# ai-dynamo/grove

Measured on AMD Instinct MI355X. Metric: podgangs_per_sec, higher is better.
Workload: dtype bf16; 1 GPU; global_batch=4, parallelism=gang1, gang_size=1, payload=2048x2048x2048x1, inflight=2, concurrent_syncs=4, transport=http, scheduler=amd-gang-scheduler (native xGMI Filter/Score)

## Files before the change

### grove_amd/kubelet/gpunode.py

```python
from __future__ import annotations

import logging
from typing import Any, Dict, Optional, Tuple

from ..api import constants as c
from ..kubecore.store import Obj

log = logging.getLogger("grove.gpunode")

PAYLOAD_ANNOTATION = "grove.io/payload"
PAYLOAD_SHAPE_ANNOTATION = "grove.io/payload-shape"
GPU_IDS_ANNOTATION = "scheduling.amd.com/gpu-ids"

_gpuwork = None


def load_gpuwork():
    global _gpuwork
    if _gpuwork is not None:
        return _gpuwork
    import torch
    try:
        from ..ops import _gpuwork as ext
    except ImportError as e:
        if torch.cuda.is_available():
            raise RuntimeError(
                "grove_amd.ops._gpuwork native extension is missing on a GPU box — "
                "build it with python -m grove_amd.ops.build") from e
        return None
    _gpuwork = ext
    return ext


PAYLOAD_KINDS = ("gemm", "stream", "decode", "decode_batch", "decode_attn")


def parse_payload_shape(kind: str, shape: str) -> Tuple[int, ...]:
    if kind == "gemm":
        dims = tuple(int(x) for x in shape.split("x")) if shape else (1024, 1024, 1024, 1)
        if len(dims) == 3:
            dims = dims + (1,)
        return dims
    if kind == "stream":
        dims = tuple(int(v) for v in shape.split("x")) if shape else (1 << 24,)
        if len(dims) == 1:
            dims = dims + (2,)
        return dims
    if kind == "decode":
        dims = tuple(int(v) for v in shape.split("x")) if shape else (8192, 8192, 4)
        if len(dims) == 2:
            dims = dims + (1,)
        return dims
    if kind == "decode_batch":
        dims = tuple(int(v) for v in shape.split("x")) if shape else (16384, 8192, 16, 4)
        if len(dims) == 3:
            dims = dims + (1,)
        if len(dims) != 4:
            raise ValueError(
                f"decode_batch payload-shape must be NxKxB[xiters], got {shape!r}")
        return dims
    if kind == "decode_attn":
        dims = tuple(int(v) for v in shape.split("x")) if shape else (64, 8, 8192, 32, 4)
        if len(dims) == 4:
            dims = dims + (1,)
        if len(dims) != 5:
            raise ValueError(
                f"decode_attn payload-shape must be HQxHKVxCTXxB[xiters], got {shape!r}")
        return dims
    raise ValueError(f"unknown payload kind {kind!r}")


def parse_payload(pod: Obj) -> Tuple[str, Tuple[int, ...]]:
    ann = pod["metadata"].get("annotations") or {}
    kind = ann.get(PAYLOAD_ANNOTATION, "gemm")
    shape = ann.get(PAYLOAD_SHAPE_ANNOTATION, "")
    if kind in PAYLOAD_KINDS:
        return kind, parse_payload_shape(kind, shape)
    return "none", ()


def assigned_gpu(pod: Obj) -> Optional[int]:
    ids = (pod["metadata"].get("annotations") or {}).get(GPU_IDS_ANNOTATION, "")
    if not ids:
        return None
    return int(ids.split(",")[0])


def run_payload_descriptor(kind: str, dims: Tuple[int, ...], device: int) -> Dict[str, Any]:
    import torch
    if not torch.cuda.is_available():
        if kind == "gemm":
            m, n, k, iters = dims
            a = torch.randn(min(m, 128), min(k, 128))
            b = torch.randn(min(k, 128), min(n, 128))
            for _ in range(iters):
                a @ b
        return {"device": "cpu", "kind": kind}
    ext = load_gpuwork()
    device = device % max(1, torch.cuda.device_count())
    with torch.cuda.device(device):
        if kind == "gemm":
            m, n, k, iters = dims
            tflops = ext.burn_gemm(m, n, k, iters)
            return {"device": device, "kind": kind, "tflops": tflops}
        if kind == "stream":
            n_floats = dims[0]
            iters = dims[1] if len(dims) > 1 else 2
            gbps = ext.stream_triad(n_floats, iters)
            return {"device": device, "kind": kind, "gbps": gbps}
        if kind == "decode":
            n, k, iters = dims
            gbps = ext.burn_decode(n, k, iters)
            return {"device": device, "kind": kind, "weight_stream_gbps": gbps}
        if kind == "decode_batch":
            n, k, batch, iters = dims
            gbps = ext.burn_decode_batch(n, k, batch, iters)
            return {"device": device, "kind": kind, "batch": batch,
                    "weight_stream_gbps": gbps,
                    "tokens_per_s": batch * gbps * 1e9 / (2.0 * n * k)}
        if kind == "decode_attn":
            hq, hkv, ctx, batch, iters = dims
            gbps = ext.burn_decode_attn(hq, hkv, ctx, batch, iters)
            kv_bytes_per_step = 2.0 * batch * hkv * ctx * 128 * 2
            return {"device": device, "kind": kind, "batch": batch, "context": ctx,
                    "kv_stream_gbps": gbps,
                    "tokens_per_s": batch * gbps * 1e9 / kv_bytes_per_step}
    return {"device": device, "kind": kind}


def gpu_pod_payload(pod: Obj) -> None:
    gpu = assigned_gpu(pod)
    kind, dims = parse_payload(pod)
    if kind == "none":
        return
    if gpu is None:
        gpu = 0
    run_payload_descriptor(kind, dims, gpu)
```

### grove_amd/ops/gpuwork.hip

```cpp
#include <torch/extension.h>
#include <ATen/hip/HIPContext.h>
#include <hip/hip_runtime.h>
#include <hip/hip_bf16.h>

#include <vector>

#define WAVE 64
#define BK 64

using bf16 = __hip_bfloat16;
using bf16x8 = __attribute__((ext_vector_type(8))) __bf16;
using f32x16 = __attribute__((ext_vector_type(16))) float;

__device__ __forceinline__ int swz(int row, int cb) {
    return (cb ^ ((row ^ (row >> 3)) & 7)) & 7;
}

__device__ __forceinline__ int lds_off(int row, int cb) {
    return row * BK + (swz(row, cb) << 3);
}

__device__ __forceinline__ void tile_map(int bid, int num_pid_m, int tiles_n,
                                         int& tile_m, int& tile_n) {
    const int GROUP = 8;
    int group_size = min(GROUP, num_pid_m);
    int pids_per_group = group_size * tiles_n;
    int group = bid / pids_per_group;
    int in_group = bid % pids_per_group;
    tile_m = group * GROUP + (in_group % group_size);
    tile_n = in_group / group_size;
}

__device__ __forceinline__ void tile_map_rect(int bid, int tiles_m, int tiles_n,
                                              int m_per_xcd, int n_win,
                                              int& tile_m, int& tile_n) {
    int mwin_tiles = 8 * m_per_xcd;
    int win = bid >> 8;
    int idx = bid & 255;
    int xcd = idx & 7;
    int slot = idx >> 3;
    int nwins = tiles_n / n_win;
    tile_m = (win / nwins) * mwin_tiles + xcd * m_per_xcd + slot % m_per_xcd;
    tile_n = (win % nwins) * n_win + slot / m_per_xcd;
}

template <int THREADS, int AUX = 0>
__device__ __forceinline__ void stage_tile(const bf16* __restrict__ g, long ld,
                                           __bf16* __restrict__ dst, int rows,
                                           int tid, int wave_piece0) {
#pragma unroll
    for (int i = 0; i < 8; ++i) {
        if (i >= (rows * 8) / THREADS)
            break;
        int p = tid + i * THREADS;
        int row = p >> 3;
        int cb_src = swz(row, p & 7);
        int base = wave_piece0 + i * THREADS;
        __builtin_amdgcn_global_load_lds(
            (const __attribute__((address_space(1))) uint32_t*)(
                g + (long)row * ld + (cb_src << 3)),
            (__attribute__((address_space(3))) uint32_t*)(dst + base * 8),
            16, 0, AUX);
    }
}

__global__ __launch_bounds__(512, 1)
void mfma_gemm_bf16_256_kernel(const bf16* __restrict__ A,
                               const bf16* __restrict__ Bt,
                               float* __restrict__ C,
                               int M, int N, int K,
                               int m_per_xcd, int n_win) {
    constexpr int BM = 256, BN = 256;
    __shared__ __bf16 smem[2 * (BM * BK + BN * BK)];
    auto sAp = [&](int b) { return smem + b * (BM * BK + BN * BK); };
    auto sBp = [&](int b) { return smem + b * (BM * BK + BN * BK) + BM * BK; };

    int tile_m, tile_n;
    if (m_per_xcd)
        tile_map_rect(blockIdx.x, M / BM, N / BN, m_per_xcd, n_win,
                      tile_m, tile_n);
    else
        tile_map(blockIdx.x, M / BM, N / BN, tile_m, tile_n);
    const int tid = threadIdx.x;
    const int wave = tid / WAVE;
    const int lane = tid % WAVE;
    const int wr = wave >> 1, wc = wave & 1;
    const long row0 = (long)tile_m * BM;
    const long col0 = (long)tile_n * BN;
    const int wave_piece0 = wave * WAVE;

    auto stage = [&](int buf, long kk) {
        stage_tile<512>(A + row0 * K + kk, K, sAp(buf), BM, tid, wave_piece0);
        stage_tile<512>(Bt + col0 * K + kk, K, sBp(buf), BN, tid, wave_piece0);
    };

    f32x16 acc[2][4] = {};
    bf16x8 afrag[2][2], bfrag[2][4];
    const int a_row = wr * 64 + (lane & 31);
    const int b_row = wc * 128 + (lane & 31);
    const int k_half = lane >> 5;
    auto load_frags = [&](int pb, int buf, int ks) {
        int cb = (ks << 1) | k_half;
#pragma unroll
        for (int mt = 0; mt < 2; ++mt)
            afrag[pb][mt] = *(const bf16x8*)(sAp(buf) + lds_off(a_row + mt * 32, cb));
#pragma unroll
        for (int nt = 0; nt < 4; ++nt)
            bfrag[pb][nt] = *(const bf16x8*)(sBp(buf) + lds_off(b_row + nt * 32, cb));
    };

    stage(0, 0);
    __syncthreads();
    load_frags(0, 0, 0);
    for (long kk = 0; kk < K; kk += BK) {
        int buf = (kk / BK) & 1;
        if (kk + BK < K) stage(buf ^ 1, kk + BK);
#pragma unroll
        for (int ks = 0; ks < BK / 16; ++ks) {
            int pb = ks & 1;
            if (ks + 1 < BK / 16)
                load_frags(pb ^ 1, buf, ks + 1);
#pragma unroll
            for (int mt = 0; mt < 2; ++mt)
#pragma unroll
                for (int nt = 0; nt < 4; ++nt)
                    acc[mt][nt] = __builtin_amdgcn_mfma_f32_32x32x16_bf16(
                        afrag[pb][mt], bfrag[pb][nt], acc[mt][nt], 0, 0, 0);
        }
        __syncthreads();
        if (kk + BK < K) load_frags(0, buf ^ 1, 0);
    }

    const int c_row_lane = 4 * (lane >> 5);
#pragma unroll
    for (int mt = 0; mt < 2; ++mt)
#pragma unroll
        for (int nt = 0; nt < 4; ++nt)
#pragma unroll
            for (int reg = 0; reg < 16; ++reg) {
                int r = wr * 64 + mt * 32 + (reg & 3) + 8 * (reg >> 2) + c_row_lane;
                int cl = wc * 128 + nt * 32 + (lane & 31);
                C[(row0 + r) * (long)N + col0 + cl] = acc[mt][nt][reg];
            }
}

__global__ __launch_bounds__(256, 2)
void mfma_gemm_bf16_128_kernel(const bf16* __restrict__ A,
                               const bf16* __restrict__ Bt,
                               float* __restrict__ C,
                               int M, int N, int K) {
    constexpr int BM = 128, BN = 128;
    __shared__ __bf16 smem[2 * (BM * BK + BN * BK)];
    auto sAp = [&](int b) { return smem + b * (BM * BK + BN * BK); };
    auto sBp = [&](int b) { return smem + b * (BM * BK + BN * BK) + BM * BK; };

    int tile_m, tile_n;
    tile_map(blockIdx.x, M / BM, N / BN, tile_m, tile_n);
    const int tid = threadIdx.x;
    const int wave = tid / WAVE;
    const int lane = tid % WAVE;
    const int wr = wave >> 1, wc = wave & 1;
    const long row0 = (long)tile_m * BM;
    const long col0 = (long)tile_n * BN;
    const int wave_piece0 = wave * WAVE;

    auto stage = [&](int buf, long kk) {
        stage_tile<256>(A + row0 * K + kk, K, sAp(buf), BM, tid, wave_piece0);
        stage_tile<256>(Bt + col0 * K + kk, K, sBp(buf), BN, tid, wave_piece0);
    };

    f32x16 acc[2][2] = {};
    bf16x8 afrag[2][2], bfrag[2][2];
    const int a_row = wr * 64 + (lane & 31);
    const int b_row = wc * 64 + (lane & 31);
    const int k_half = lane >> 5;
    auto load_frags = [&](int pb, int buf, int ks) {
        int cb = (ks << 1) | k_half;
#pragma unroll
        for (int mt = 0; mt < 2; ++mt)
            afrag[pb][mt] = *(const bf16x8*)(sAp(buf) + lds_off(a_row + mt * 32, cb));
#pragma unroll
        for (int nt = 0; nt < 2; ++nt)
            bfrag[pb][nt] = *(const bf16x8*)(sBp(buf) + lds_off(b_row + nt * 32, cb));
    };

    stage(0, 0);
    __syncthreads();
    load_frags(0, 0, 0);
    for (long kk = 0; kk < K; kk += BK) {
        int buf = (kk / BK) & 1;
        if (kk + BK < K) stage(buf ^ 1, kk + BK);
#pragma unroll
        for (int ks = 0; ks < BK / 16; ++ks) {
            int pb = ks & 1;
            if (ks + 1 < BK / 16)
                load_frags(pb ^ 1, buf, ks + 1);
#pragma unroll
            for (int mt = 0; mt < 2; ++mt)
#pragma unroll
                for (int nt = 0; nt < 2; ++nt)
                    acc[mt][nt] = __builtin_amdgcn_mfma_f32_32x32x16_bf16(
                        afrag[pb][mt], bfrag[pb][nt], acc[mt][nt], 0, 0, 0);
        }
        __syncthreads();
        if (kk + BK < K) load_frags(0, buf ^ 1, 0);
    }

    const int c_row_lane = 4 * (lane >> 5);
#pragma unroll
    for (int mt = 0; mt < 2; ++mt)
#pragma unroll
        for (int nt = 0; nt < 2; ++nt)
#pragma unroll
            for (int reg = 0; reg < 16; ++reg) {
                int r = wr * 64 + mt * 32 + (reg & 3) + 8 * (reg >> 2) + c_row_lane;
                int cl = wc * 64 + nt * 32 + (lane & 31);
                C[(row0 + r) * (long)N + col0 + cl] = acc[mt][nt][reg];
            }
}

__global__ __launch_bounds__(256)
void decode_gemv_kernel(const bf16* __restrict__ W,
                        const bf16* __restrict__ x,
                        float* __restrict__ y, int N, int K) {
    const int lane = threadIdx.x % WAVE;
    const int wave = threadIdx.x / WAVE;
    const int row = blockIdx.x * 4 + wave;
    if (row >= N) return;
    const bf16* w = W + (long)row * K;
    float acc = 0.f;
    for (int k0 = lane * 8; k0 < K; k0 += WAVE * 8) {
        bf16x8 wv = *(const bf16x8*)(w + k0);
        bf16x8 xv = *(const bf16x8*)(x + k0);
#pragma unroll
        for (int i = 0; i < 8; ++i)
            acc += (float)wv[i] * (float)xv[i];
    }
    for (int off = 32; off > 0; off >>= 1)
        acc += __shfl_down(acc, off, 64);
    if (lane == 0) y[row] = acc;
}

torch::Tensor decode_gemv(torch::Tensor w, torch::Tensor x) {
    TORCH_CHECK(w.is_cuda() && x.is_cuda() && w.dtype() == torch::kBFloat16
                && x.dtype() == torch::kBFloat16, "bf16 GPU tensors required");
    TORCH_CHECK(w.is_contiguous() && x.is_contiguous(), "contiguous required");
    int64_t N = w.size(0), K = w.size(1);
    TORCH_CHECK(x.numel() == K && K % 512 == 0, "x must be [K], K%512==0");
    auto y = torch::empty({N}, w.options().dtype(torch::kFloat32));
    hipStream_t stream = at::hip::getCurrentHIPStream();
    hipLaunchKernelGGL(decode_gemv_kernel, dim3((N + 3) / 4), dim3(256), 0, stream,
                       (const bf16*)w.data_ptr(), (const bf16*)x.data_ptr(),
                       y.data_ptr<float>(), (int)N, (int)K);
    return y;
}

double burn_decode(int64_t n, int64_t k, int64_t iters) {
    auto opt = torch::TensorOptions().dtype(torch::kBFloat16).device(torch::kCUDA);
    auto w = torch::randn({n, k}, opt.dtype(torch::kFloat32)).to(torch::kBFloat16);
    auto x = torch::randn({k}, opt.dtype(torch::kFloat32)).to(torch::kBFloat16);
    auto y = torch::empty({n}, opt.dtype(torch::kFloat32));
    hipStream_t stream = at::hip::getCurrentHIPStream();
    auto launch = [&] {
        hipLaunchKernelGGL(decode_gemv_kernel, dim3((n + 3) / 4), dim3(256), 0,
                           stream, (const bf16*)w.data_ptr(),
                           (const bf16*)x.data_ptr(), y.data_ptr<float>(),
                           (int)n, (int)k);
    };
    launch();
    C10_HIP_CHECK(hipStreamSynchronize(stream));
    auto t0 = std::chrono::steady_clock::now();
    for (int64_t i = 0; i < iters; ++i) launch();
    C10_HIP_CHECK(hipStreamSynchronize(stream));
    auto t1 = std::chrono::steady_clock::now();
    double secs = std::chrono::duration<double>(t1 - t0).count();
    return 2.0 * n * k * iters / secs / 1e9;
}

using f32x4 = __attribute__((ext_vector_type(4))) float;

#define DG_STEP 128

template <int T, int R>
__global__ __launch_bounds__(256)
void decode_gemm_kernel(const bf16* __restrict__ W,
                        const bf16* __restrict__ X,
                        float* __restrict__ Y,
                        int B, int N, int K) {
    __shared__ f32x4 red[4 * R * T * WAVE];
    const int lane = threadIdx.x % WAVE;
    const int wave = threadIdx.x / WAVE;
    const int r = lane & 15, g = lane >> 4;
    const int kq = K / 4;
    const int steps = kq / DG_STEP;
    const long koff = (long)wave * kq + 8 * g;
    const long n0 = (long)blockIdx.x * (16 * R);
    const bf16* wp = W + (n0 + r) * K + koff;
    const auto xrsrc = __builtin_amdgcn_make_buffer_rsrc(
        const_cast<bf16*>(X), 0, B * K * 2, 0x00020000);
    unsigned xoff[T];
#pragma unroll
    for (int t = 0; t < T; ++t)
        xoff[t] = (unsigned)(((long)(t * 16 + r) * K + koff) * 2);

    auto load_w = [&](bf16x8 (&w)[R][4], int s) {
#pragma unroll
        for (int q = 0; q < R; ++q) {
            const bf16x8* p = (const bf16x8*)(wp + (long)q * 16 * K + (long)s * DG_STEP);
#pragma unroll
            for (int i = 0; i < 4; ++i)
                w[q][i] = p[4 * i];
        }
    };
    auto load_x = [&](bf16x8 (&x)[T][4], int s) {
#pragma unroll
        for (int t = 0; t < T; ++t)
#pragma unroll
            for (int i = 0; i < 4; ++i)
                x[t][i] = __builtin_bit_cast(bf16x8, __builtin_amdgcn_raw_buffer_load_b128(
                    xrsrc, xoff[t] + s * (DG_STEP * 2) + i * 64, 0, 0));
    };

    f32x4 acc[R][T] = {};
    auto mma = [&](const bf16x8 (&w)[R][4], const bf16x8 (&x)[T][4]) {
#pragma unroll
        for (int i = 0; i < 4; ++i)
#pragma unroll
            for (int q = 0; q < R; ++q)
#pragma unroll
                for (int t = 0; t < T; ++t)
                    acc[q][t] = __builtin_amdgcn_mfma_f32_16x16x32_bf16(
                        w[q][i], x[t][i], acc[q][t], 0, 0, 0);
    };

    bf16x8 w0[R][4], w1[R][4], xf[T][4];
    load_w(w0, 0);
    int s = 0;
    for (; s + 2 < steps; s += 2) {
        load_x(xf, s);
        load_w(w1, s + 1);
        mma(w0, xf);
        load_x(xf, s + 1);
        load_w(w0, s + 2);
        mma(w1, xf);
    }
    load_x(xf, s);
    if (s + 1 < steps) {
        load_w(w1, s + 1);
        mma(w0, xf);
        load_x(xf, s + 1);
        mma(w1, xf);
    } else {
        mma(w0, xf);
    }

#pragma unroll
    for (int q = 0; q < R; ++q)
#pragma unroll
        for (int t = 0; t < T; ++t)
            red[((wave * R + q) * T + t) * WAVE + lane] = acc[q][t];
    __syncthreads();
    const int nl = threadIdx.x & 15, bl = threadIdx.x >> 4;
    const float* redf = (const float*)red;
    const int src = (((nl >> 2) * 16 + bl) << 2) + (nl & 3);
#pragma unroll
    for (int q = 0; q < R; ++q)
#pragma unroll
        for (int t = 0; t < T; ++t) {
            int b = t * 16 + bl;
            if (b < B) {
                float sum = redf[(q * T + t) * WAVE * 4 + src];
#pragma unroll
                for (int w = 1; w < 4; ++w)
                    sum += redf[((w * R + q) * T + t) * WAVE * 4 + src];
                Y[(long)b * N + n0 + q * 16 + nl] = sum;
            }
        }
}

static void check_decode_gemm_dims(int64_t B, int64_t N, int64_t K) {
    TORCH_CHECK(B >= 1 && B <= 64 && N >= 16 && N % 16 == 0 && K >= 512 && K % 512 == 0
                && N <= INT32_MAX && K <= (1 << 23),
                "decode_gemm_bf16 requires 1<=B<=64, N%16==0, K%512==0 (got B=", B,
                " N=", N, " K=", K, ")");
}

template <int T>
static void launch_decode_gemm_t(const bf16* w, const bf16* x, float* y, int B, int N,
                                 int K, int rows, hipStream_t stream) {
    dim3 grid(N / (16 * rows)), block(256);
    auto go = [&](auto kernel) {
        hipLaunchKernelGGL(kernel, grid, block, 0, stream, w, x, y, B, N, K);
    };
    if (rows == 4) go(decode_gemm_kernel<T, 4>);
    else if (rows == 2) go(decode_gemm_kernel<T, 2>);
    else go(decode_gemm_kernel<T, 1>);
}

static int decode_gemm_rows(int64_t B, int64_t N) {
    int rows = B <= 8 ? 1 : B <= 16 ? 2 : 4;
    while (rows > 1 && (N % (16 * rows) != 0 || N / (16 * rows) < 256))
        rows /= 2;
    return rows;
}

static void launch_decode_gemm(const bf16* w, const bf16* x, float* y, int64_t B,
                               int64_t N, int64_t K, int64_t rows, hipStream_t stream) {
    if (!rows) rows = decode_gemm_rows(B, N);
    TORCH_CHECK((rows == 1 || rows == 2 || rows == 4) && N % (16 * rows) == 0,
                "rows must be 0 (auto), 1, 2 or 4 and 16*rows must divide N");
    switch ((B + 15) / 16) {
    case 1: launch_decode_gemm_t<1>(w, x, y, B, N, K, rows, stream); break;
    case 2: launch_decode_gemm_t<2>(w, x, y, B, N, K, rows, stream); break;
    case 3: launch_decode_gemm_t<3>(w, x, y, B, N, K, rows, stream); break;
    default: launch_decode_gemm_t<4>(w, x, y, B, N, K, rows, stream); break;
    }
}

torch::Tensor decode_gemm_bf16(torch::Tensor w, torch::Tensor x) {
    TORCH_CHECK(w.is_cuda() && x.is_cuda() && w.dtype() == torch::kBFloat16
                && x.dtype() == torch::kBFloat16, "bf16 GPU tensors required");
    TORCH_CHECK(w.get_device() == x.get_device(), "w and x must be on one device");
    TORCH_CHECK(w.dim() == 2 && x.dim() == 2, "w must be [N,K] and x [B,K]");
    TORCH_CHECK(w.is_contiguous() && x.is_contiguous(), "contiguous required");
    int64_t N = w.size(0), K = w.size(1), B = x.size(0);
    TORCH_CHECK(x.size(1) == K, "shape mismatch: w[N,K] x[B,K]");
    check_decode_gemm_dims(B, N, K);
    auto y = torch::empty({B, N}, w.options().dtype(torch::kFloat32));
    launch_decode_gemm((const bf16*)w.data_ptr(), (const bf16*)x.data_ptr(),
                       y.data_ptr<float>(), B, N, K, 0,
                       at::hip::getCurrentHIPStream());
    return y;
}

double burn_decode_batch(int64_t n, int64_t k, int64_t batch, int64_t iters,
                         int64_t rows) {
    check_decode_gemm_dims(batch, n, k);
    auto opt = torch::TensorOptions().dtype(torch::kBFloat16).device(torch::kCUDA);
    auto w = torch::randn({n, k}, opt.dtype(torch::kFloat32)).to(torch::kBFloat16);
    auto x = torch::randn({batch, k}, opt.dtype(torch::kFloat32)).to(torch::kBFloat16);
    auto y = torch::empty({batch, n}, opt.dtype(torch::kFloat32));
    hipStream_t stream = at::hip::getCurrentHIPStream();
    auto launch = [&] {
        launch_decode_gemm((const bf16*)w.data_ptr(), (const bf16*)x.data_ptr(),
                           y.data_ptr<float>(), batch, n, k, rows, stream);
    };
    launch();
    C10_HIP_CHECK(hipStreamSynchronize(stream));
    auto t0 = std::chrono::steady_clock::now();
    for (int64_t i = 0; i < iters; ++i) launch();
    C10_HIP_CHECK(hipStreamSynchronize(stream));
    auto t1 = std::chrono::steady_clock::now();
    double secs = std::chrono::duration<double>(t1 - t0).count();
    return 2.0 * n * k * iters / secs / 1e9;
}

__global__ void stream_triad_kernel(const float4* __restrict__ a,
                                    const float4* __restrict__ b,
                                    float4* __restrict__ c, long n4, float s) {
    long i = (long)blockIdx.x * blockDim.x + threadIdx.x;
    long stride = (long)gridDim.x * blockDim.x;
    for (; i < n4; i += stride) {
        float4 x = a[i], y = b[i];
        c[i] = make_float4(x.x + s * y.x, x.y + s * y.y, x.z + s * y.z, x.w + s * y.w);
    }
}


static void launch_gemm(const torch::Tensor& a, const torch::Tensor& bt,
                        torch::Tensor& c, int64_t M, int64_t N, int64_t K,
                        int64_t map_mode = -1) {
    hipStream_t stream = at::hip::getCurrentHIPStream();
    if (M % 256 == 0 && N % 256 == 0 && (M / 256) * (N / 256) >= 256) {
        int tiles_m = (int)(M / 256), tiles_n = (int)(N / 256);
        int m_per_xcd = 0, n_win = 0;
        int mpx = std::min<int>(4, std::max(1, tiles_m / 8));
        int nw = 256 / (8 * mpx);
        bool want_rect = (map_mode == 1) ||
                         (map_mode < 0 && (int64_t)tiles_m * tiles_n > 256);
        if (want_rect && map_mode != 0 &&
            tiles_m % (8 * mpx) == 0 && tiles_n % nw == 0) {
            m_per_xcd = mpx; n_win = nw;
        }
        dim3 grid((M / 256) * (N / 256)), block(512);
        hipLaunchKernelGGL(mfma_gemm_bf16_256_kernel, grid, block, 0, stream,
                           (const bf16*)a.data_ptr(), (const bf16*)bt.data_ptr(),
                           c.data_ptr<float>(), (int)M, (int)N, (int)K,
                           m_per_xcd, n_win);
    } else {
        dim3 grid((M / 128) * (N / 128)), block(256);
        hipLaunchKernelGGL(mfma_gemm_bf16_128_kernel, grid, block, 0, stream,
                           (const bf16*)a.data_ptr(), (const bf16*)bt.data_ptr(),
                           c.data_ptr<float>(), (int)M, (int)N, (int)K);
    }
}

static void check_dims(int64_t M, int64_t N, int64_t K) {
    TORCH_CHECK(M % 128 == 0 && N % 128 == 0 && K % 64 == 0,
                "mfma_gemm_bf16 requires M%128==0, N%128==0, K%64==0 (got ",
                M, "x", N, "x", K, ")");
}

torch::Tensor mfma_gemm_bf16(torch::Tensor a, torch::Tensor bt) {
    TORCH_CHECK(a.is_cuda() && bt.is_cuda(), "inputs must be on GPU");
    TORCH_CHECK(a.dtype() == torch::kBFloat16 && bt.dtype() == torch::kBFloat16,
                "inputs must be bf16");
    TORCH_CHECK(a.is_contiguous() && bt.is_contiguous(), "inputs must be contiguous");
    int64_t M = a.size(0), K = a.size(1), N = bt.size(0);
    TORCH_CHECK(bt.size(1) == K, "shape mismatch: A[M,K] Bt[N,K]");
    check_dims(M, N, K);
    auto c = torch::empty({M, N}, a.options().dtype(torch::kFloat32));
    launch_gemm(a, bt, c, M, N, K);
    return c;
}

double burn_gemm(int64_t m, int64_t n, int64_t k, int64_t iters,
                 int64_t map_mode) {
    check_dims(m, n, k);
    auto opt = torch::TensorOptions().dtype(torch::kBFloat16).device(torch::kCUDA);
    auto a = torch::randn({m, k}, opt.dtype(torch::kFloat32)).to(torch::kBFloat16);
    auto bt = torch::randn({n, k}, opt.dtype(torch::kFloat32)).to(torch::kBFloat16);
    auto c = torch::empty({m, n}, opt.dtype(torch::kFloat32));
    hipStream_t stream = at::hip::getCurrentHIPStream();
    launch_gemm(a, bt, c, m, n, k, map_mode);
    C10_HIP_CHECK(hipStreamSynchronize(stream));
    auto t0 = std::chrono::steady_clock::now();
    for (int64_t i = 0; i < iters; ++i) launch_gemm(a, bt, c, m, n, k, map_mode);
    C10_HIP_CHECK(hipStreamSynchronize(stream));
    auto t1 = std::chrono::steady_clock::now();
    double secs = std::chrono::duration<double>(t1 - t0).count();
    return 2.0 * m * n * k * iters / secs / 1e12;
}

double stream_triad(int64_t n_floats, int64_t iters) {
    TORCH_CHECK(n_floats % 4 == 0, "n_floats must be a multiple of 4");
    auto opt = torch::TensorOptions().dtype(torch::kFloat32).device(torch::kCUDA);
    auto a = torch::randn({n_floats}, opt);
    auto b = torch::randn({n_floats}, opt);
    auto c = torch::empty({n_floats}, opt);
    long n4 = n_floats / 4;
    hipStream_t stream = at::hip::getCurrentHIPStream();
    int blocks = std::min<long>(8192, (n4 + 255) / 256);
    auto launch = [&] {
        hipLaunchKernelGGL(stream_triad_kernel, dim3(blocks), dim3(256), 0, stream,
                           (const float4*)a.data_ptr(), (const float4*)b.data_ptr(),
                           (float4*)c.data_ptr(), n4, 1.5f);
    };
    launch();
    C10_HIP_CHECK(hipStreamSynchronize(stream));
    auto t0 = std::chrono::steady_clock::now();
    for (int64_t i = 0; i < iters; ++i) launch();
    C10_HIP_CHECK(hipStreamSynchronize(stream));
    auto t1 = std::chrono::steady_clock::now();
    double secs = std::chrono::duration<double>(t1 - t0).count();
    return 12.0 * n_floats * iters / secs / 1e9;
}

torch::Tensor decode_attn_bf16(torch::Tensor q, torch::Tensor k_cache,
                               torch::Tensor v_cache, torch::Tensor seq_lens,
                               double scale, int64_t splits);
int64_t decode_attn_splits(int64_t batch, int64_t hkv, int64_t lmax);
double burn_decode_attn(int64_t hq, int64_t hkv, int64_t ctx, int64_t batch,
                        int64_t iters, int64_t splits);

PYBIND11_MODULE(TORCH_EXTENSION_NAME, m) {
    m.doc() = "grove_amd MI355X pod-payload kernels (MFMA bf16 GEMM, HBM stream, "
              "decode GEMV, batched decode skinny GEMM, split-KV decode attention)";
    m.def("mfma_gemm_bf16", &mfma_gemm_bf16, "C[M,N]=A[M,K]@Bt[N,K]^T (bf16 in, fp32 out)");
    m.def("burn_gemm", &burn_gemm, "run iters GEMM steps; returns TFLOP/s",
          pybind11::arg("m"), pybind11::arg("n"), pybind11::arg("k"),
          pybind11::arg("iters"), pybind11::arg("map_mode") = -1);
    m.def("burn_gemm_v",
          [](int64_t m_, int64_t n_, int64_t k_, int64_t it, int64_t) {
              return burn_gemm(m_, n_, k_, it, -1);
          }, "compat alias for burn_gemm (bk arg ignored)");
    m.def("stream_triad", &stream_triad, "HBM triad; returns GB/s");
    m.def("decode_gemv", &decode_gemv, "y[N]=W[N,K]@x[K] (bf16 in, fp32 out)");
    m.def("burn_decode", &burn_decode,
          "iters decode GEMV steps; returns weight-stream GB/s");
    m.def("decode_gemm_bf16", &decode_gemm_bf16,
          "y[B,N]=x[B,K]@W[N,K]^T for 1<=B<=64, N%16==0, K%512==0 "
          "(args w, x; bf16 in, fp32 out)");
    m.def("burn_decode_batch", &burn_decode_batch,
          "iters batched decode steps; returns weight-stream GB/s",
          pybind11::arg("n"), pybind11::arg("k"), pybind11::arg("batch"),
          pybind11::arg("iters"), pybind11::arg("rows") = 0);
    m.def("decode_attn_bf16", &decode_attn_bf16,
          "out[B,Hq,128]=softmax(scale*q.k^T).v over k/v_cache[B,Hkv,Lmax,128] up to "
          "seq_lens[B] (int32, on device); bf16 in, fp32 out; scale=0 -> 1/sqrt(128); "
          "splits=0 -> automatic",
          pybind11::arg("q"), pybind11::arg("k_cache"), pybind11::arg("v_cache"),
          pybind11::arg("seq_lens"), pybind11::arg("scale") = 0.0,
          pybind11::arg("splits") = 0);
    m.def("decode_attn_splits", &decode_attn_splits,
          "KV splits decode_attn_bf16 picks for a shape",
          pybind11::arg("batch"), pybind11::arg("hkv"), pybind11::arg("lmax"));
    m.def("burn_decode_attn", &burn_decode_attn,
          "iters decode-attention steps; returns KV-stream GB/s",
          pybind11::arg("hq"), pybind11::arg("hkv"), pybind11::arg("ctx"),
          pybind11::arg("batch"), pybind11::arg("iters"), pybind11::arg("splits") = 0);
}
```

Measured before the change: 358.4 gangs/s.

## Run pod payloads in native code with fused fill, no warmup, GIL released

Adds native payload entry points for gemm, decode and decode_batch. Each one fills both operands with a single counter-hash bf16 kernel into one shared buffer, runs the iterations without a warmup launch, and synchronises once. These calls release the GIL and pick the device with a C++ guard instead of the Python torch.cuda.device context. The aim is to drop the torch.randn plus cast kernels, the warmup GEMM and the extra syncs, and to let concurrent pod syncs overlap. In exchange the input distribution changes from normal to uniform, and timing now includes the fill.

Measured after the change: 332.2 gangs/s. 7.3% lower.

```diff
diff --git a/grove_amd/kubelet/gpunode.py b/grove_amd/kubelet/gpunode.py
--- a/grove_amd/kubelet/gpunode.py
+++ b/grove_amd/kubelet/gpunode.py
@@ -98,26 +98,26 @@
         return {"device": "cpu", "kind": kind}
     ext = load_gpuwork()
     device = device % max(1, torch.cuda.device_count())
+    if kind == "gemm":
+        m, n, k, iters = dims
+        tflops = ext.gemm_payload(m, n, k, iters, device)
+        return {"device": device, "kind": kind, "tflops": tflops}
+    if kind == "decode":
+        n, k, iters = dims
+        gbps = ext.decode_payload(n, k, iters, device)
+        return {"device": device, "kind": kind, "weight_stream_gbps": gbps}
+    if kind == "decode_batch":
+        n, k, batch, iters = dims
+        gbps = ext.decode_batch_payload(n, k, batch, iters, device)
+        return {"device": device, "kind": kind, "batch": batch,
+                "weight_stream_gbps": gbps,
+                "tokens_per_s": batch * gbps * 1e9 / (2.0 * n * k)}
     with torch.cuda.device(device):
-        if kind == "gemm":
-            m, n, k, iters = dims
-            tflops = ext.burn_gemm(m, n, k, iters)
-            return {"device": device, "kind": kind, "tflops": tflops}
         if kind == "stream":
             n_floats = dims[0]
             iters = dims[1] if len(dims) > 1 else 2
             gbps = ext.stream_triad(n_floats, iters)
             return {"device": device, "kind": kind, "gbps": gbps}
-        if kind == "decode":
-            n, k, iters = dims
-            gbps = ext.burn_decode(n, k, iters)
-            return {"device": device, "kind": kind, "weight_stream_gbps": gbps}
-        if kind == "decode_batch":
-            n, k, batch, iters = dims
-            gbps = ext.burn_decode_batch(n, k, batch, iters)
-            return {"device": device, "kind": kind, "batch": batch,
-                    "weight_stream_gbps": gbps,
-                    "tokens_per_s": batch * gbps * 1e9 / (2.0 * n * k)}
         if kind == "decode_attn":
             hq, hkv, ctx, batch, iters = dims
             gbps = ext.burn_decode_attn(hq, hkv, ctx, batch, iters)
diff --git a/grove_amd/ops/gpuwork.hip b/grove_amd/ops/gpuwork.hip
--- a/grove_amd/ops/gpuwork.hip
+++ b/grove_amd/ops/gpuwork.hip
@@ -2,7 +2,12 @@
 #include <ATen/hip/HIPContext.h>
 #include <hip/hip_runtime.h>
 #include <hip/hip_bf16.h>
-
+#include <c10/core/DeviceGuard.h>
+#include <c10/hip/HIPFunctions.h>
+
+#include <atomic>
+#include <chrono>
+#include <variant>
 #include <vector>
 
 #define WAVE 64
@@ -532,6 +537,167 @@
     return 2.0 * m * n * k * iters / secs / 1e12;
 }
 
+
+__device__ __forceinline__ uint32_t mix32(uint32_t x) {
+    x ^= x >> 16; x *= 0x7feb352dU;
+    x ^= x >> 15; x *= 0x846ca68bU;
+    x ^= x >> 16;
+    return x;
+}
+
+__device__ __forceinline__ uint32_t bf16_bits_rne(float f) {
+    uint32_t u = __float_as_uint(f);
+    return (u + 0x7fffu + ((u >> 16) & 1u)) >> 16;
+}
+
+__global__ __launch_bounds__(256)
+void fill_random_bf16_kernel(uint4* __restrict__ out, long n8, uint32_t key0,
+                             uint32_t key1) {
+    long i = (long)blockIdx.x * blockDim.x + threadIdx.x;
+    const long stride = (long)gridDim.x * blockDim.x;
+    for (; i < n8; i += stride) {
+        uint32_t w[4];
+#pragma unroll
+        for (int j = 0; j < 4; ++j) {
+            unsigned long p = (unsigned long)i * 4 + j;
+            uint32_t h = mix32(mix32((uint32_t)p ^ key0) + (uint32_t)(p >> 32) + key1);
+            float lo = ((float)(int)(h & 0xffffu) - 32768.f) * (1.f / 16384.f);
+            float hi = ((float)(int)(h >> 16) - 32768.f) * (1.f / 16384.f);
+            w[j] = bf16_bits_rne(lo) | (bf16_bits_rne(hi) << 16);
+        }
+        out[i] = make_uint4(w[0], w[1], w[2], w[3]);
+    }
+}
+
+static uint64_t splitmix64(uint64_t x) {
+    x += 0x9e3779b97f4a7c15ULL;
+    x = (x ^ (x >> 30)) * 0xbf58476d1ce4e5b9ULL;
+    x = (x ^ (x >> 27)) * 0x94d049bb133111ebULL;
+    return x ^ (x >> 31);
+}
+
+static uint64_t resolve_seed(int64_t seed) {
+    if (seed != 0) return (uint64_t)seed;
+    static std::atomic<uint64_t> counter{1};
+    uint64_t tick = (uint64_t)std::chrono::steady_clock::now().time_since_epoch().count();
+    return splitmix64(counter.fetch_add(1, std::memory_order_relaxed) ^ (tick << 20)) | 1;
+}
+
+static void launch_fill(const torch::Tensor& t, uint64_t seed, hipStream_t stream) {
+    long n8 = t.numel() / 8;
+    if (n8 == 0) return;
+    uint64_t key = splitmix64(seed);
+    int blocks = (int)std::min<long>(2048, (n8 + 255) / 256);
+    hipLaunchKernelGGL(fill_random_bf16_kernel, dim3(blocks), dim3(256), 0, stream,
+                       (uint4*)t.data_ptr(), n8, (uint32_t)key, (uint32_t)(key >> 32));
+}
+
+void fill_random_bf16(torch::Tensor t, int64_t seed) {
+    TORCH_CHECK(t.is_cuda() && t.dtype() == torch::kBFloat16, "bf16 GPU tensor required");
+    TORCH_CHECK(t.is_contiguous(), "contiguous tensor required");
+    TORCH_CHECK(t.numel() % 8 == 0, "numel must be a multiple of 8 (got ", t.numel(), ")");
+    TORCH_CHECK((uintptr_t)t.data_ptr() % 16 == 0, "data must be 16-byte aligned");
+    c10::DeviceGuard guard(t.device());
+    launch_fill(t, resolve_seed(seed), at::hip::getCurrentHIPStream());
+}
+
+static void select_device(c10::OptionalDeviceGuard& guard, int64_t device) {
+    if (device < 0) return;
+    TORCH_CHECK(device < (int64_t)c10::hip::device_count(), "no GPU ", device);
+    guard.reset_device(c10::Device(c10::kCUDA, (c10::DeviceIndex)device));
+}
+
+struct PayloadOperands {
+    torch::Tensor buf, a, b;
+};
+
+static PayloadOperands payload_operands(int64_t rows_a, int64_t rows_b, int64_t k,
+                                        uint64_t seed, hipStream_t stream) {
+    TORCH_CHECK(rows_a >= 1 && rows_b >= 1 && k >= 8 && k % 8 == 0,
+                "payload operands need rows >= 1 and k % 8 == 0 (got ", rows_a, "+",
+                rows_b, " rows, k=", k, ")");
+    auto opt = torch::TensorOptions().dtype(torch::kBFloat16).device(torch::kCUDA);
+    PayloadOperands o;
+    o.buf = torch::empty({rows_a + rows_b, k}, opt);
+    o.a = o.buf.narrow(0, 0, rows_a);
+    o.b = o.buf.narrow(0, rows_a, rows_b);
+    launch_fill(o.buf, seed, stream);
+    return o;
+}
+
+std::vector<torch::Tensor> payload_inputs(int64_t m, int64_t n, int64_t k, int64_t seed) {
+    auto o = payload_operands(m, n, k, resolve_seed(seed), at::hip::getCurrentHIPStream());
+    return {o.a, o.b};
+}
+
+using PayloadResult = std::variant<double, torch::Tensor>;
+
+PayloadResult gemm_payload(int64_t m, int64_t n, int64_t k, int64_t iters,
+                           int64_t device, int64_t seed, bool return_product) {
+    check_dims(m, n, k);
+    TORCH_CHECK(m > 0 && n > 0 && k > 0 && iters >= 0, "positive dims required");
+    c10::OptionalDeviceGuard guard;
+    select_device(guard, device);
+    hipStream_t stream = at::hip::getCurrentHIPStream();
+    auto c = torch::empty({m, n}, torch::TensorOptions().dtype(torch::kFloat32)
+                                      .device(torch::kCUDA));
+    auto t0 = std::chrono::steady_clock::now();
+    auto o = payload_operands(m, n, k, resolve_seed(seed), stream);
+    for (int64_t i = 0; i < iters; ++i) launch_gemm(o.a, o.b, c, m, n, k);
+    C10_HIP_CHECK(hipGetLastError());
+    C10_HIP_CHECK(hipStreamSynchronize(stream));
+    auto t1 = std::chrono::steady_clock::now();
+    if (return_product) return c;
+    double secs = std::chrono::duration<double>(t1 - t0).count();
+    return 2.0 * m * n * k * iters / secs / 1e12;
+}
+
+PayloadResult decode_payload(int64_t n, int64_t k, int64_t iters, int64_t device,
+                             int64_t seed, bool return_product) {
+    TORCH_CHECK(n >= 1 && n <= INT32_MAX - 3 && k >= 512 && k % 512 == 0
+                && k <= INT32_MAX && iters >= 0,
+                "decode payload requires N>=1, K%512==0 (got N=", n, " K=", k, ")");
+    c10::OptionalDeviceGuard guard;
+    select_device(guard, device);
+    hipStream_t stream = at::hip::getCurrentHIPStream();
+    auto y = torch::empty({n}, torch::TensorOptions().dtype(torch::kFloat32)
+                                   .device(torch::kCUDA));
+    auto t0 = std::chrono::steady_clock::now();
+    auto o = payload_operands(n, 1, k, resolve_seed(seed), stream);
+    for (int64_t i = 0; i < iters; ++i)
+        hipLaunchKernelGGL(decode_gemv_kernel, dim3((n + 3) / 4), dim3(256), 0, stream,
+                           (const bf16*)o.a.data_ptr(), (const bf16*)o.b.data_ptr(),
+                           y.data_ptr<float>(), (int)n, (int)k);
+    C10_HIP_CHECK(hipGetLastError());
+    C10_HIP_CHECK(hipStreamSynchronize(stream));
+    auto t1 = std::chrono::steady_clock::now();
+    if (return_product) return y;
+    double secs = std::chrono::duration<double>(t1 - t0).count();
+    return 2.0 * n * k * iters / secs / 1e9;
+}
+
+PayloadResult decode_batch_payload(int64_t n, int64_t k, int64_t batch, int64_t iters,
+                                   int64_t device, int64_t seed, bool return_product) {
+    check_decode_gemm_dims(batch, n, k);
+    TORCH_CHECK(iters >= 0, "iters must not be negative");
+    c10::OptionalDeviceGuard guard;
+    select_device(guard, device);
+    hipStream_t stream = at::hip::getCurrentHIPStream();
+    auto y = torch::empty({batch, n}, torch::TensorOptions().dtype(torch::kFloat32)
+                                          .device(torch::kCUDA));
+    auto t0 = std::chrono::steady_clock::now();
+    auto o = payload_operands(n, batch, k, resolve_seed(seed), stream);
+    for (int64_t i = 0; i < iters; ++i)
+        launch_decode_gemm((const bf16*)o.a.data_ptr(), (const bf16*)o.b.data_ptr(),
+                           y.data_ptr<float>(), batch, n, k, 0, stream);
+    C10_HIP_CHECK(hipGetLastError());
+    C10_HIP_CHECK(hipStreamSynchronize(stream));
+    auto t1 = std::chrono::steady_clock::now();
+    if (return_product) return y;
+    double secs = std::chrono::duration<double>(t1 - t0).count();
+    return 2.0 * n * k * iters / secs / 1e9;
+}
+
 double stream_triad(int64_t n_floats, int64_t iters) {
     TORCH_CHECK(n_floats % 4 == 0, "n_floats must be a multiple of 4");
     auto opt = torch::TensorOptions().dtype(torch::kFloat32).device(torch::kCUDA);
@@ -574,6 +740,36 @@
           [](int64_t m_, int64_t n_, int64_t k_, int64_t it, int64_t) {
               return burn_gemm(m_, n_, k_, it, -1);
           }, "compat alias for burn_gemm (bk arg ignored)");
+    m.def("fill_random_bf16", &fill_random_bf16,
+          "fill a contiguous 16-B-aligned bf16 tensor (numel%8==0) with uniform "
+          "[-2,2) values that depend only on (seed, index); seed 0 = fresh seed",
+          pybind11::arg("tensor"), pybind11::arg("seed") = 0);
+    m.def("payload_inputs", &payload_inputs,
+          "the (A[m,k], Bt[n,k]) a payload call with this seed uses",
+          pybind11::arg("m"), pybind11::arg("n"), pybind11::arg("k"),
+          pybind11::arg("seed"));
+    m.def("gemm_payload", &gemm_payload,
+          "pod payload: one fill, iters GEMMs, one sync; returns TFLOP/s (or C with "
+          "return_product); runs with the GIL released",
+          pybind11::arg("m"), pybind11::arg("n"), pybind11::arg("k"),
+          pybind11::arg("iters"), pybind11::arg("device") = -1,
+          pybind11::arg("seed") = 0, pybind11::arg("return_product") = false,
+          pybind11::call_guard<pybind11::gil_scoped_release>());
+    m.def("decode_payload", &decode_payload,
+          "pod payload: one fill, iters decode GEMVs, one sync; returns weight-stream "
+          "GB/s (or y[n] with return_product); runs with the GIL released",
+          pybind11::arg("n"), pybind11::arg("k"), pybind11::arg("iters"),
+          pybind11::arg("device") = -1, pybind11::arg("seed") = 0,
+          pybind11::arg("return_product") = false,
+          pybind11::call_guard<pybind11::gil_scoped_release>());
+    m.def("decode_batch_payload", &decode_batch_payload,
+          "pod payload: one fill, iters batched decode steps, one sync; returns "
+          "weight-stream GB/s (or y[batch,n] with return_product); runs with the GIL "
+          "released",
+          pybind11::arg("n"), pybind11::arg("k"), pybind11::arg("batch"),
+          pybind11::arg("iters"), pybind11::arg("device") = -1,
+          pybind11::arg("seed") = 0, pybind11::arg("return_product") = false,
+          pybind11::call_guard<pybind11::gil_scoped_release>());
     m.def("stream_triad", &stream_triad, "HBM triad; returns GB/s");
     m.def("decode_gemv", &decode_gemv, "y[N]=W[N,K]@x[K] (bf16 in, fp32 out)");
     m.def("burn_decode", &burn_decode,
```
